# rfahrn/RadVLM

Hardware: AMD Instinct MI355X
Metric: train image-instruction pairs/sec, LLaVA-1.5-7B 336px (higher is better)
Workload: dtype bf16; 1 GPU; llava15_7b full fine-tune step (ViT frozen): fwd+bwd+AdamW, S=704, 32 pairs/GPU/step; global_batch=32, seq_len=704, parallelism=dp1, rows_with_a_label_only=last layer's o_proj / norm / MLP, final norm, lm_head, cross entropy

## Files before the change

include/radvlm_hip.h:

```cpp
#ifndef RADVLM_HIP_H
#define RADVLM_HIP_H
#include <stdint.h>

#ifdef __cplusplus
extern "C" {
#endif

#define RV_ACT_NONE 0
#define RV_ACT_QUICK_GELU 1
#define RV_ACT_GELU 2
#define RV_ACT_GELU_TANH 3

const char* rv_version(void);

int rv_gemm_nt_bf16(const void* A, int64_t lda, const void* B, int64_t ldb, void* C, int64_t ldc, const void* bias,
                    const void* residual, int64_t ldr, int M, int N, int K, int act, int out_f32, int res_f32,
                    const void* zeros16, void* stream);
int rv_gemm_bf16(const void* A, int64_t lda, const void* B, int64_t ldb, void* C, int64_t ldc, const void* bias,
                 const void* residual, int64_t ldr, int M, int N, int K, int trans_a, int trans_b, float alpha, int act,
                 int out_f32, int res_f32, const void* zeros16, void* stream);
int rv_gemm_bf16_ex(const void* A, int64_t lda, const void* B, int64_t ldb, void* C, int64_t ldc, const void* bias,
                    const void* residual, int64_t ldr, int M, int N, int K, int trans_a, int trans_b, float alpha, int act,
                    int out_f32, int res_f32, const void* A2, int64_t lda2, const void* B2, int64_t ldb2, int K2,
                    void* workspace, int64_t workspace_bytes, const void* zeros16, void* stream);
// ... 54 lines not shown
                    int S_pad, int hd, int causal, float scale, void* workspace, int64_t workspace_bytes, const void* zeros16,
                    void* stream);
int rv_attn_bwd_gqa_rope(const void* q, int64_t ld_q, const void* k, int64_t ld_k, const void* v, int64_t ld_v, const void* o,
                         int64_t ld_o, const void* dout, int64_t ld_do, const void* qT, const void* kT, const void* doT,
                         const float* lse, float* delta, void* dq, int64_t ld_dq, void* dk, int64_t ld_dk, void* dv,
                         int64_t ld_dv, const int32_t* lens, const int32_t* cu_rows, int total_rows, int B, int H, int H_kv, int S,
                         int S_pad, int hd, int causal, float scale, void* workspace, int64_t workspace_bytes,
                         const float* rope_cos_sin, const int32_t* rope_positions, const void* zeros16, void* stream);

int rv_attn_bwd_nat(const void* q, int64_t ld_q, const void* k, int64_t ld_k, const void* v, int64_t ld_v, const void* o, int64_t ld_o,
                    const void* dout, int64_t ld_do, const float* lse, float* delta, void* dq, int64_t ld_dq, void* dk, int64_t ld_dk,
                    void* dv, int64_t ld_dv, const int32_t* lens, const int32_t* cu_rows, int total_rows, int B, int H, int H_kv, int S,
                    int S_pad, int hd, int causal, float scale, void* workspace, int64_t workspace_bytes, const float* rope_cos_sin,
                    const int32_t* rope_positions, const void* zeros16, void* stream);

int rv_transpose_bf16_varlen(const void* in, int64_t in_ld, const int32_t* cu_rows, int64_t in_bs1, void* out, int64_t out_ld,
                             int64_t out_bs0, int64_t out_bs1, int R_max, int C, int R_pad, int nb0, int nb1, int perm32,
                             void* stream);
int rv_rope_inplace_pos(void* x, int64_t ld, const float* cos_sin, const int32_t* positions, int rows, int heads, int hd,
                        int nsec, int dir, void* stream);

int rv_swiglu_fwd(const void* gu, int64_t ld_gu, void* act, int64_t ld_act, int rows, int F, void* stream);
int rv_swiglu_bwd(const void* dact, int64_t ld_dact, const void* gu, int64_t ld_gu, void* dgu, int64_t ld_dgu, int rows,
                  int F, void* stream);
int rv_dropout_bf16(const void* x, void* y, int64_t n, float p, uint64_t seed, void* stream);
int rv_dropout_add_bf16(const void* x, void* y, int64_t n, float p, uint64_t seed, void* stream);
int rv_gemm_dropout_add_bf16(const void* A, int64_t lda, const void* B, int64_t ldb, void* C, int64_t ldc, int M, int N, int K, int trans_b,
                             float alpha, float p, uint64_t seed, int accumulate, const void* zeros16, void* stream);
int rv_lora_down_bf16(const void* X, int64_t ldx, const void* A, int64_t lda, void* T, int64_t ldt, int M, int R, int K, float alpha,
                      float p, uint64_t seed, const void* zeros16, void* stream);
// ... 66 lines not shown
```

radvlm_amd/csrc/attention.hip:

```cpp
#include <type_traits>
#include <stdlib.h>
#include "common.h"
#include "radvlm_hip.h"

struct AttnParams {
    const bf16 *q, *k, *v, *o, *dout;
    const bf16 *qT, *kT, *vT, *doT;
    bf16 *out, *dq, *dk, *dv;
    float *lse, *delta;
    const int* lens;
    const int* cu;
    const bf16* zeros;
    long ld_q, ld_k, ld_v, ld_o, ld_do, ld_dq, ld_dk, ld_dv;
    int B, H, S, S_pad;
    int kdiv, qrep;
    int Hkv, nrep;
    float scale;
    const float* rope_cs; const int* rope_pos;
    int paired;
    int rope_dk;
};

namespace {

// ... 54 lines not shown
    return __builtin_amdgcn_make_buffer_rsrc((void*)base, 0, (unsigned)(rows * row_stride * 2), 0x00020000);
}

DEVINL bf16x8 tf_get(const TFrag& f) {
    typedef __attribute__((ext_vector_type(8))) short s16x8n;
    const s16x8n r = {f.t0[0], f.t0[1], f.t0[2], f.t0[3], f.t1[0], f.t1[1], f.t1[2], f.t1[3]};
    return __builtin_bit_cast(bf16x8, r);
}
template <int LEFT> DEVINL void lds_wait8(bf16x8 (&a)[4], bf16x8 (&b)[4]) {
    asm volatile("s_waitcnt lgkmcnt(%8)" : "+v"(a[0]), "+v"(a[1]), "+v"(a[2]), "+v"(a[3]), "+v"(b[0]), "+v"(b[1]), "+v"(b[2]), "+v"(b[3]) : "i"(LEFT) : "memory");
}
template <int LEFT> DEVINL void tf_wait8(TFrag (&f)[4], TFrag (&h)[4]) {
    asm volatile("s_waitcnt lgkmcnt(%16)" : "+v"(f[0].t0), "+v"(f[0].t1), "+v"(f[1].t0), "+v"(f[1].t1), "+v"(f[2].t0), "+v"(f[2].t1), "+v"(f[3].t0), "+v"(f[3].t1),
                   "+v"(h[0].t0), "+v"(h[0].t1), "+v"(h[1].t0), "+v"(h[1].t1), "+v"(h[2].t0), "+v"(h[2].t1), "+v"(h[3].t0), "+v"(h[3].t1) : "i"(LEFT) : "memory");
}
template <int LEFT> DEVINL void tf_wait4(TFrag (&f)[4]) {
    asm volatile("s_waitcnt lgkmcnt(%8)" : "+v"(f[0].t0), "+v"(f[0].t1), "+v"(f[1].t0), "+v"(f[1].t1), "+v"(f[2].t0), "+v"(f[2].t1), "+v"(f[3].t0), "+v"(f[3].t1)
                 : "i"(LEFT) : "memory");
}

template <bool HEAVY_LAST_FIRST>
DEVINL void block_coords(int& xb, int& h, int& b) {
    const int gx = gridDim.x, gy = gridDim.y;
    const int lin = blockIdx.x + gx * (blockIdx.y + gy * blockIdx.z);
    const int pid = xcd_remap(lin, gx * gy * (int)gridDim.z);
    const int hh = pid / gx;
    xb = pid - hh * gx;
    if (HEAVY_LAST_FIRST) xb = gx - 1 - xb;
    h = hh % gy;
    b = hh / gy;
}

template <int N, class F>
DEVINL void sfor(F&& f) {
    if constexpr (N > 0) {
        sfor<N - 1>(f);
        f(std::integral_constant<int, N - 1>{});
    }
}
struct NatAddr {
    unsigned row[4], col[8];
    DEVINL void init(const char* image, int lane) {
        const int g = lane >> 4, c = lane & 15, r1 = (lane >> 2) & 15, pp = lane & 3;
        const unsigned b = lds_off(image);
#pragma unroll
        for (int ks = 0; ks < 4; ++ks) row[ks] = b + c * 256 + (((ks * 4 + g) ^ nswz(c)) << 4);
#pragma unroll
        for (int db = 0; db < 8; ++db) col[db] = b + r1 * 256 + (((2 * db + (pp >> 1)) ^ nswz(r1)) << 4) + ((pp & 1) << 3);
    }
    DEVINL void shift(int delta) {
#pragma unroll
        for (int i = 0; i < 4; ++i) row[i] += delta;
#pragma unroll
        for (int i = 0; i < 8; ++i) col[i] += delta;
    }
};
template <int IMM> DEVINL void rdrow_imm(bf16x8& dst, unsigned a) {
    asm volatile("ds_read_b128 %0, %1 offset:%2" : "=v"(dst) : "v"(a), "i"(IMM) : "memory");
}
template <int IMM> DEVINL void rdcol_imm(TFrag& f, unsigned a) {
    asm volatile("ds_read_b64_tr_b16 %0, %1 offset:%2" : "=v"(f.t0) : "v"(a), "i"(IMM) : "memory");
    asm volatile("ds_read_b64_tr_b16 %0, %1 offset:%2" : "=v"(f.t1) : "v"(a), "i"(IMM + 4096) : "memory");
}
DEVINL float max3_asm(float a, float b, float c) { float r; asm volatile("v_max3_f32 %0, %1, %2, %3" : "=v"(r) : "v"(a), "v"(b), "v"(c)); return r; }

template <int ROW_BYTES> DEVINL int swz(int r) { return ROW_BYTES == 128 ? ((r >> 1) & 7) : (r & 15); }

template <int ROW_BYTES, int NROWS, int NW = 4>
DEVINL void stage_rows(const bf16* src, long row_stride, int valid_rows, const bf16* zeros, char* lds, int wid, int lane) {
    constexpr int CPR = ROW_BYTES / 16;
// ... 619 lines not shown
    for (; t < ntiles; ++t) tile(t, std::false_type{});
#pragma unroll
    for (int qs = 0; qs < 2; ++qs) {
        const int qidx = q0 + qs * 16 + c;
        if (qidx >= S) continue;
        bf16* op = P.dq + (rb + qidx) * P.ld_dq + h * HD + 4 * g;
        f32x4 v[DB];
#pragma unroll
        for (int db = 0; db < DB; ++db) v[db] = dq[qs][db] * P.scale;
        if (P.rope_cs) unrope<DB>(v, P.rope_cs + (long)(P.rope_pos ? P.rope_pos[rb + qidx] : qidx) * HD, g);
#pragma unroll
        for (int db = 0; db < DB; ++db) *(bf16x4*)(op + db * 16) = bf16x4{f2bf(v[db][0]), f2bf(v[db][1]), f2bf(v[db][2]), f2bf(v[db][3])};
    }
}

template <bool CAUSAL, int NW>
__global__ __launch_bounds__(NW * 64, 2) void attn_bwd_dkv_nat_kernel(AttnParams P) {
    constexpr int HD = 128, KS = 4, DB = 8, TILE = 64 * 256, STAGE = 2 * TILE + 1024;
    extern __shared__ __attribute__((aligned(16))) char smem[];
    const int wid = wave_id(), lane = lane_id(), g = lane >> 4, c = lane & 15;
    int kblk, h, b;
    block_coords<false>(kblk, h, b);
    constexpr int KPB = NW * 16;
    const long rb = P.cu ? (long)P.cu[b] : (long)b * P.S;
    const int S = P.cu ? P.cu[b + 1] - P.cu[b] : P.S, k0 = kblk * KPB + wid * 16;
    if (kblk * KPB >= S) return;
    const int len = (P.lens && !P.cu) ? P.lens[b] : S;
    const float sl2 = P.scale * LOG2E;

    bf16x8 kf[KS], vf[KS];
    {
        const int row = min(k0 + c, S - 1);
        const bf16* kp = P.k + (rb + row) * P.ld_k + (h / P.kdiv) * HD + g * 8;
        const bf16* vp = P.v + (rb + row) * P.ld_v + (h / P.kdiv) * HD + g * 8;
#pragma unroll
        for (int ks = 0; ks < KS; ++ks) { kf[ks] = *(const bf16x8*)(kp + ks * 32); vf[ks] = *(const bf16x8*)(vp + ks * 32); }
    }
    const int q_end = len;
    const int t0 = CAUSAL ? (kblk * KPB) >> 6 : 0;
    const int t1 = (q_end + 63) >> 6;
    const int nt = max(t1 - t0, 0);
    const int n_it = nt * P.qrep;

    f32x4 dv[DB], dk[DB];
#pragma unroll
    for (int db = 0; db < DB; ++db) { dv[db] = f32x4{0.f, 0.f, 0.f, 0.f}; dk[db] = f32x4{0.f, 0.f, 0.f, 0.f}; }

    const __amdgpu_buffer_rsrc_t rsQ = rows_rsrc(P.q + rb * P.ld_q, S, P.ld_q), rsO = rows_rsrc(P.dout + rb * P.ld_do, S, P.ld_do);
    NatPlan<64, NW> plQ, plO;
    plQ.init(P.ld_q, wid, lane);
    plO.init(P.ld_do, wid, lane);
    auto stage = [&](int it, char* dst) {
        const int hq = h * P.qrep + it / nt;
        const int qt0 = (t0 + it % nt) * 64;
        const float* lsebase = P.lse + (long)(b * P.H + hq) * P.S_pad;
        const float* dlbase = P.delta + (long)(b * P.H + hq) * P.S_pad;
        plQ.stage(rsQ, (int)((long)qt0 * P.ld_q * 2) + hq * HD * 2, dst, wid);
        plO.stage(rsO, (int)((long)qt0 * P.ld_do * 2) + hq * HD * 2, dst + TILE, wid);
        if (wid == 0) {
            const float* gp = lane < 16 ? lsebase + qt0 + lane * 4 : (lane < 32 ? dlbase + qt0 + (lane - 16) * 4 : (const float*)P.zeros);
            glds16(gp, dst + 2 * TILE);
        }
    };
    if (n_it > 0) stage(0, smem);
    NatAddr ad;
    ad.init(smem + STAGE, lane);

    auto iter = [&](int it, int j, auto edge_tag) {
        constexpr bool EDGE = decltype(edge_tag)::value;
        asm volatile("s_waitcnt vmcnt(0)" ::: "memory");
        __syncthreads();
        ad.shift((it & 1) ? STAGE : -STAGE);
        const char* LSt = smem + (it & 1) * STAGE + 2 * TILE;
        if (it + 1 < n_it) stage(it + 1, smem + ((it + 1) & 1) * STAGE);
        const int qt0 = (t0 + j) * 64;
        if (EDGE && CAUSAL && qt0 + 63 < k0) return;
        {
            sfor<2>([&](auto qpt) {
                constexpr int qp = decltype(qpt)::value;
                if (EDGE && CAUSAL && qt0 + qp * 32 + 31 < k0) return;
                TFrag dc[2][4], qc[2][4];
                auto issue_c = [&](auto bit, TFrag (&dd)[4], TFrag (&qd)[4]) {
                    constexpr int bi = decltype(bit)::value;
                    sfor<4>([&](auto u) {
                        rdcol_imm<TILE + qp * 8192>(dd[decltype(u)::value], ad.col[bi * 4 + decltype(u)::value]);
                        rdcol_imm<qp * 8192>(qd[decltype(u)::value], ad.col[bi * 4 + decltype(u)::value]);
                    });
                };
                f32x4 s[2], dp[2];
                s[0] = s[1] = dp[0] = dp[1] = f32x4{0.f, 0.f, 0.f, 0.f};
                bf16x8 qa[2][KS], da[2][KS];
                sfor<2>([&](auto qq) {
                    sfor<KS>([&](auto ks) {
                        rdrow_imm<(2 * qp + decltype(qq)::value) * 4096>(qa[decltype(qq)::value][decltype(ks)::value], ad.row[decltype(ks)::value]);
                        rdrow_imm<TILE + (2 * qp + decltype(qq)::value) * 4096>(da[decltype(qq)::value][decltype(ks)::value], ad.row[decltype(ks)::value]);
                    });
                });
                lds_wait8<2 * KS>(qa[0], da[0]);
                __builtin_amdgcn_sched_barrier(0);
#pragma unroll
                for (int ks = 0; ks < KS; ++ks) { s[0] = mfma16(qa[0][ks], kf[ks], s[0]); dp[0] = mfma16(da[0][ks], vf[ks], dp[0]); }
                __builtin_amdgcn_sched_barrier(0);
                issue_c(std::integral_constant<int, 0>{}, dc[0], qc[0]);
                lds_wait8<15>(qa[1], da[1]);
                __builtin_amdgcn_sched_barrier(0);
#pragma unroll
                for (int ks = 0; ks < KS; ++ks) { s[1] = mfma16(qa[1][ks], kf[ks], s[1]); dp[1] = mfma16(da[1][ks], vf[ks], dp[1]); }
                __builtin_amdgcn_sched_barrier(0);
#pragma unroll
                for (int qq = 0; qq < 2; ++qq) {
                    const int qrow = qt0 + (2 * qp + qq) * 16 + 4 * g;
                    const f32x4 ls = *(const f32x4*)(LSt + (qrow - qt0) * 4);
                    const f32x4 dl = *(const f32x4*)(LSt + 256 + (qrow - qt0) * 4);
                    const int kidx = k0 + c;
#pragma unroll
                    for (int r = 0; r < 4; ++r) {
                        float p = fexp2(__builtin_fmaf(s[qq][r], sl2, -ls[r] * LOG2E));
                        if (EDGE) {
                            const int qidx = qrow + r;
                            p = ((kidx < len) && (qidx < q_end) && (!CAUSAL || kidx <= qidx)) ? p : 0.f;
                        }
                        s[qq][r] = p;
                        dp[qq][r] = p * (dp[qq][r] - dl[r]);
                    }
                }
                const bf16x8 pf = pack8(s[0], s[1]), dsf = pack8(dp[0], dp[1]);
                sfor<2>([&](auto bit) {
                    constexpr int bi = decltype(bit)::value;
                    if constexpr (bi == 0) { issue_c(std::integral_constant<int, 1>{}, dc[1], qc[1]); tf_wait8<15>(dc[0], qc[0]); }
                    else tf_wait8<0>(dc[1], qc[1]);
                    __builtin_amdgcn_sched_barrier(0);
#pragma unroll
                    for (int u = 0; u < 4; ++u) {
                        dv[bi * 4 + u] = mfma16(tf_get(dc[bi][u]), pf, dv[bi * 4 + u]);
                        dk[bi * 4 + u] = mfma16(tf_get(qc[bi][u]), dsf, dk[bi * 4 + u]);
                    }
                    __builtin_amdgcn_sched_barrier(0);
                });
            });
        }
    };
    {
        const bool key_partial = kblk * KPB + KPB > len;
        const int ne0 = key_partial ? nt : (CAUSAL ? min(nt, (KPB + 63) / 64) : 0);
        const int ni = max(ne0, min(nt, (q_end >> 6) - t0));
        int it = 0;
        for (int rep = 0; rep < P.qrep; ++rep) {
            for (int j = 0; j < ne0; ++j, ++it) iter(it, j, std::true_type{});
            for (int j = ne0; j < ni; ++j, ++it) iter(it, j, std::false_type{});
            for (int j = ni; j < nt; ++j, ++it) iter(it, j, std::true_type{});
        }
    }
    {
        const int kidx = k0 + c;
        if (kidx < S) {
            bf16* vp = P.dv + (rb + kidx) * P.ld_dv + h * HD + 4 * g;
            bf16* kp = P.dk + (rb + kidx) * P.ld_dk + h * HD + 4 * g;
            f32x4 kk[DB];
#pragma unroll
            for (int db = 0; db < DB; ++db) kk[db] = dk[db] * P.scale;
            if (P.rope_cs && P.rope_dk) unrope<DB>(kk, P.rope_cs + (long)(P.rope_pos ? P.rope_pos[rb + kidx] : kidx) * HD, g);
#pragma unroll
            for (int db = 0; db < DB; ++db) {
                const f32x4 a = dv[db];
                *(bf16x4*)(vp + db * 16) = bf16x4{f2bf(a[0]), f2bf(a[1]), f2bf(a[2]), f2bf(a[3])};
                *(bf16x4*)(kp + db * 16) = bf16x4{f2bf(kk[db][0]), f2bf(kk[db][1]), f2bf(kk[db][2]), f2bf(kk[db][3])};
            }
        }
    }
}

template <int HD, bool CAUSAL, int NW>
__global__ __launch_bounds__(NW * 64, NW / 4) void attn_bwd_dq_kernel(AttnParams P) {
    constexpr int KS = HD / 32, DB = HD / 16, KROW = HD * 2;
    constexpr int NAT_BYTES = 64 * KROW, T_BYTES = HD * 128, STAGE = 2 * NAT_BYTES + T_BYTES;
    extern __shared__ __attribute__((aligned(16))) char smem[];
    const int wid = wave_id(), lane = lane_id(), g = lane >> 4, c = lane & 15;
    const int qblk = blockIdx.x, h = blockIdx.y, b = blockIdx.z;
    const long rb = P.cu ? (long)P.cu[b] : (long)b * P.S;
// ... 315 lines not shown
    } while (0)
    if (HD == 128) { if (causal) LAUNCH_FWD(128, true); else LAUNCH_FWD(128, false); }
    else { if (causal) LAUNCH_FWD(64, true); else LAUNCH_FWD(64, false); }
#undef LAUNCH_FWD
    return rv_check_launch();
}

namespace {
template __global__ void attn_fwd_nat_kernel<true>(AttnParams);
template __global__ void attn_fwd_nat_kernel<false>(AttnParams);
#ifndef RV_DQ_NW
#define RV_DQ_NW 4
#endif
template __global__ void attn_bwd_dq_nat_kernel<true, RV_DQ_NW>(AttnParams);
template __global__ void attn_bwd_dq_nat_kernel<false, RV_DQ_NW>(AttnParams);
template __global__ void attn_bwd_dkv_nat_kernel<true, 4>(AttnParams);
template __global__ void attn_bwd_dkv_nat_kernel<false, 4>(AttnParams);
}

static int g_attn_cus() {
    static int cus = 0;
    if (!cus) {
        int dev = 0, n = 0;
        if (hipGetDevice(&dev) == hipSuccess && hipDeviceGetAttribute(&n, hipDeviceAttributeMultiprocessorCount, dev) == hipSuccess && n > 0) cus = n;
        else cus = 256;
    }
    return cus;
}
static int attn_fwd_pairs(int B, int H, int S, int causal) {
    const int nq = (S + 127) / 128;
    const long pairs = (long)((nq + 1) / 2) * H * B;
    const long slots = 2L * g_attn_cus();
// ... 80 lines not shown
    } while (0)
    if (HD == 128) { if (causal) LAUNCH_BWD(128, true); else LAUNCH_BWD(128, false); }
    else { if (causal) LAUNCH_BWD(64, true); else LAUNCH_BWD(64, false); }
#undef LAUNCH_BWD
    if (expand) {
        const long rows = rows_all, total = rows * (H_kv * HD / 16);
        hipLaunchKernelGGL(group_sum_heads_kernel, dim3((total + 255) / 256), dim3(256), 0, st, PK.dk, PK.ld_dk, P.dk, P.ld_dk, rows, H_kv, P.nrep, HD,
                           rope_cos_sin, rope_positions, cu_rows, S);
        hipLaunchKernelGGL(group_sum_heads_kernel, dim3((total + 255) / 256), dim3(256), 0, st, PK.dv, PK.ld_dv, P.dv, P.ld_dv, rows, H_kv, P.nrep, HD,
                           (const float*)nullptr, (const int32_t*)nullptr, cu_rows, S);
    }
    return rv_check_launch();
}


extern "C" int rv_attn_bwd_nat(const void* q, int64_t ld_q, const void* k, int64_t ld_k, const void* v, int64_t ld_v, const void* o, int64_t ld_o,
                               const void* dout, int64_t ld_do, const float* lse, float* delta, void* dq, int64_t ld_dq, void* dk, int64_t ld_dk,
                               void* dv, int64_t ld_dv, const int32_t* lens, const int32_t* cu_rows, int total_rows, int B, int H, int H_kv, int S,
                               int S_pad, int HD, int causal, float scale, void* workspace, int64_t workspace_bytes, const float* rope_cos_sin,
                               const int32_t* rope_positions, const void* zeros16, void* stream) {
    if (!q || !k || !v || !o || !dout || !lse || !delta || !dq || !dk || !dv || !zeros16) return RV_ERR_ARG;
    if (H_kv <= 0 || H <= 0 || H % H_kv || HD != 128 || (S_pad & 63) || S_pad < S || B <= 0 || S <= 0) return RV_ERR_ARG;
    if ((ld_q & 7) || (ld_k & 7) || (ld_v & 7) || (ld_do & 7) || (ld_o & 7) || (ld_dq & 3) || (ld_dk & 3) || (ld_dv & 3)) return RV_ERR_ARG;
    if (!aligned_ok(q) || !aligned_ok(k) || !aligned_ok(v) || !aligned_ok(dout) || !aligned_ok(o)) return RV_ERR_ARG;
    if (rope_cos_sin && ((((uintptr_t)rope_cos_sin) & 15) || (cu_rows && !rope_positions))) return RV_ERR_ARG;
    AttnParams P = {};
    P.q = (const bf16*)q; P.k = (const bf16*)k; P.v = (const bf16*)v; P.o = (const bf16*)o; P.dout = (const bf16*)dout;
    P.dq = (bf16*)dq; P.dk = (bf16*)dk; P.dv = (bf16*)dv; P.lse = (float*)lse; P.delta = delta; P.lens = lens; P.cu = cu_rows;
    P.zeros = (const bf16*)zeros16;
    P.ld_q = ld_q; P.ld_k = ld_k; P.ld_v = ld_v; P.ld_o = ld_o; P.ld_do = ld_do; P.ld_dq = ld_dq; P.ld_dk = ld_dk; P.ld_dv = ld_dv;
    P.B = B; P.H = H; P.S = S; P.S_pad = S_pad; P.scale = scale; P.Hkv = H_kv; P.nrep = H / H_kv;
    P.rope_cs = rope_cos_sin; P.rope_pos = rope_positions; P.rope_dk = 1;
    hipStream_t st = (hipStream_t)stream;
    dim3 grid_dq((S + 32 * RV_DQ_NW - 1) / (32 * RV_DQ_NW), H, B), grid_dkv((S + 63) / 64, H_kv, B);
    AttnParams PK = P;
    PK.kdiv = 1; PK.qrep = P.nrep;
    const long rows_all = cu_rows ? (long)total_rows : (long)B * S;
    if (cu_rows && total_rows <= 0) return RV_ERR_ARG;
    const int64_t need = 2 * (int64_t)rows_all * H * HD * 2;
    const bool expand = P.nrep > 1 && workspace && workspace_bytes >= need && (((uintptr_t)workspace) & 15) == 0 &&
                        (long)grid_dkv.x * H_kv * B < 4096;
    if (expand) {
        PK.kdiv = P.nrep; PK.qrep = 1; PK.rope_dk = 0;
        PK.dk = (bf16*)workspace; PK.dv = (bf16*)workspace + (int64_t)rows_all * H * HD;
        PK.ld_dk = PK.ld_dv = (long)H * HD;
        grid_dkv.y = H;
    }
    const int smem_dq = 2 * 2 * 64 * 256, smem_dkv = 2 * (2 * 64 * 256 + 1024);
#define LAUNCH_BWD_NAT(C_)                                                                                 \
    do {                                                                                                   \
        set_smem(attn_bwd_dq_nat_kernel<C_, RV_DQ_NW>, smem_dq);                                                  \
        set_smem(attn_bwd_dkv_nat_kernel<C_, 4>, smem_dkv);                                                \
        hipLaunchKernelGGL((attn_bwd_dq_nat_kernel<C_, RV_DQ_NW>), grid_dq, dim3(64 * RV_DQ_NW), smem_dq, st, P);           \
        hipLaunchKernelGGL((attn_bwd_dkv_nat_kernel<C_, 4>), grid_dkv, dim3(256), smem_dkv, st, PK);       \
    } while (0)
    if (causal) LAUNCH_BWD_NAT(true); else LAUNCH_BWD_NAT(false);
#undef LAUNCH_BWD_NAT
    if (expand) {
        const long total = rows_all * (H_kv * HD / 16);
        hipLaunchKernelGGL(group_sum_heads_kernel, dim3((total + 255) / 256), dim3(256), 0, st, PK.dk, PK.ld_dk, P.dk, P.ld_dk, rows_all, H_kv, P.nrep, HD,
                           rope_cos_sin, rope_positions, cu_rows, S);
        hipLaunchKernelGGL(group_sum_heads_kernel, dim3((total + 255) / 256), dim3(256), 0, st, PK.dv, PK.ld_dv, P.dv, P.ld_dv, rows_all, H_kv, P.nrep, HD,
                           (const float*)nullptr, (const int32_t*)nullptr, cu_rows, S);
    }
    return rv_check_launch();
}

extern "C" int rv_attn_bwd_gqa(const void* q, int64_t ld_q, const void* k, int64_t ld_k, const void* v, int64_t ld_v,
                               const void* o, int64_t ld_o, const void* dout, int64_t ld_do, const void* qT, const void* kT,
                               const void* doT, const float* lse, float* delta, void* dq, int64_t ld_dq, void* dk,
                               int64_t ld_dk, void* dv, int64_t ld_dv, const int32_t* lens, const int32_t* cu_rows, int total_rows,
                               int B, int H, int H_kv, int S, int S_pad, int HD, int causal, float scale, void* workspace, int64_t workspace_bytes,
                               const void* zeros16, void* stream) {
    return rv_attn_bwd_gqa_rope(q, ld_q, k, ld_k, v, ld_v, o, ld_o, dout, ld_do, qT, kT, doT, lse, delta, dq, ld_dq, dk, ld_dk, dv, ld_dv,
                                lens, cu_rows, total_rows, B, H, H_kv, S, S_pad, HD, causal, scale, workspace, workspace_bytes, nullptr, nullptr,
                                zeros16, stream);
}

extern "C" int rv_attn_bwd(const void* q, int64_t ld_q, const void* k, int64_t ld_k, const void* v, int64_t ld_v,
                           const void* o, int64_t ld_o, const void* dout, int64_t ld_do, const void* qT, const void* kT,
// ... 7 lines not shown
```

radvlm_amd/lib.py:

```python
import ctypes
import os

import torch

_HERE = os.path.dirname(os.path.abspath(__file__))
_LIB_PATH = os.path.join(_HERE, "libradvlm_hip.so")

_c_void_p = ctypes.c_void_p
_i64 = ctypes.c_int64
_i32 = ctypes.c_int
_f32 = ctypes.c_float

ACT_NONE, ACT_QUICK_GELU, ACT_GELU, ACT_GELU_TANH = 0, 1, 2, 3

_SIGS = {
    "rv_gemm_nt_bf16": [_c_void_p, _i64, _c_void_p, _i64, _c_void_p, _i64, _c_void_p, _c_void_p, _i64, _i32, _i32, _i32,
                        _i32, _i32, _i32, _c_void_p, _c_void_p],
    "rv_gemm_bf16": [_c_void_p, _i64, _c_void_p, _i64, _c_void_p, _i64, _c_void_p, _c_void_p, _i64, _i32, _i32, _i32, _i32, _i32,
                     _f32, _i32, _i32, _i32, _c_void_p, _c_void_p],
    "rv_gemm_bf16_ex": [_c_void_p, _i64, _c_void_p, _i64, _c_void_p, _i64, _c_void_p, _c_void_p, _i64, _i32, _i32, _i32, _i32, _i32,
                        _f32, _i32, _i32, _i32, _c_void_p, _i64, _c_void_p, _i64, _i32, _c_void_p, _i64, _c_void_p, _c_void_p],
    "rv_gemm_rope_bf16": [_c_void_p, _i64, _c_void_p, _i64, _c_void_p, _i64, _c_void_p, _i32, _i32, _i32, _c_void_p, _c_void_p, _i32, _i32, _i32,
                          _c_void_p, _i64, _c_void_p, _c_void_p],
    "rv_gemm_swiglu_fwd_bf16": [_c_void_p, _i64, _c_void_p, _i64, _c_void_p, _i64, _c_void_p, _i64, _i32, _i32, _i32, _c_void_p, _i64, _c_void_p,
# ... 19 lines not shown
    "rv_attn_fwd": [_c_void_p, _i64, _c_void_p, _i64, _c_void_p, _c_void_p, _i64, _c_void_p, _c_void_p, _i32, _i32, _i32, _i32,
                    _i32, _i32, _f32, _c_void_p, _c_void_p],
    "rv_attn_bwd": [_c_void_p, _i64, _c_void_p, _i64, _c_void_p, _i64, _c_void_p, _i64, _c_void_p, _i64, _c_void_p, _c_void_p,
                    _c_void_p, _c_void_p, _c_void_p, _c_void_p, _i64, _c_void_p, _i64, _c_void_p, _i64, _c_void_p, _i32, _i32,
                    _i32, _i32, _i32, _i32, _f32, _c_void_p, _c_void_p],
    "rv_attn_fwd_gqa": [_c_void_p, _i64, _c_void_p, _i64, _c_void_p, _c_void_p, _i64, _c_void_p, _c_void_p, _c_void_p, _i32, _i32, _i32,
                        _i32, _i32, _i32, _i32, _f32, _c_void_p, _c_void_p],
    "rv_attn_bwd_gqa": [_c_void_p, _i64, _c_void_p, _i64, _c_void_p, _i64, _c_void_p, _i64, _c_void_p, _i64, _c_void_p, _c_void_p,
                        _c_void_p, _c_void_p, _c_void_p, _c_void_p, _i64, _c_void_p, _i64, _c_void_p, _i64, _c_void_p, _c_void_p, _i32,
                        _i32, _i32, _i32, _i32, _i32, _i32, _i32, _f32, _c_void_p, _i64, _c_void_p, _c_void_p],
    "rv_attn_fwd_nat": [_c_void_p, _i64, _c_void_p, _i64, _c_void_p, _i64, _c_void_p, _i64, _c_void_p, _c_void_p, _c_void_p, _i32, _i32, _i32,
                        _i32, _i32, _i32, _i32, _f32, _c_void_p, _c_void_p],
    "rv_attn_bwd_nat": [_c_void_p, _i64, _c_void_p, _i64, _c_void_p, _i64, _c_void_p, _i64, _c_void_p, _i64, _c_void_p, _c_void_p, _c_void_p, _i64,
                        _c_void_p, _i64, _c_void_p, _i64, _c_void_p, _c_void_p, _i32, _i32, _i32, _i32, _i32, _i32, _i32, _i32, _f32, _c_void_p, _i64,
                        _c_void_p, _c_void_p, _c_void_p, _c_void_p],
    "rv_attn_bwd_gqa_rope": [_c_void_p, _i64, _c_void_p, _i64, _c_void_p, _i64, _c_void_p, _i64, _c_void_p, _i64, _c_void_p, _c_void_p,
                             _c_void_p, _c_void_p, _c_void_p, _c_void_p, _i64, _c_void_p, _i64, _c_void_p, _i64, _c_void_p, _c_void_p, _i32,
                             _i32, _i32, _i32, _i32, _i32, _i32, _i32, _f32, _c_void_p, _i64, _c_void_p, _c_void_p, _c_void_p, _c_void_p],
    "rv_transpose_bf16_varlen": [_c_void_p, _i64, _c_void_p, _i64, _c_void_p, _i64, _i64, _i64, _i32, _i32, _i32, _i32, _i32, _i32,
                                 _c_void_p],
    "rv_rope_inplace_pos": [_c_void_p, _i64, _c_void_p, _c_void_p, _i32, _i32, _i32, _i32, _i32, _c_void_p],
    "rv_gelu_tanh_fwd": [_c_void_p, _c_void_p, _i64, _c_void_p],
    "rv_gelu_tanh_bwd": [_c_void_p, _c_void_p, _c_void_p, _i64, _c_void_p],
    "rv_weighted_segment_sum_rows": [_c_void_p, _i64, _c_void_p, _c_void_p, _c_void_p, _c_void_p, _i32, _c_void_p, _i64, _i32,
                                     _c_void_p],
    "rv_max4_rows_fwd": [_c_void_p, _i64, _c_void_p, _c_void_p, _i32, _c_void_p, _i64, _c_void_p, _i32, _c_void_p],
    "rv_max4_rows_bwd": [_c_void_p, _i64, _c_void_p, _c_void_p, _i32, _c_void_p, _c_void_p, _i64, _i32, _c_void_p],
    "rv_add_pos_rows": [_c_void_p, _c_void_p, _i32, _i32, _i32, _c_void_p],
    "rv_swiglu_fwd": [_c_void_p, _i64, _c_void_p, _i64, _i32, _i32, _c_void_p],
    "rv_swiglu_bwd": [_c_void_p, _i64, _c_void_p, _i64, _c_void_p, _i64, _i32, _i32, _c_void_p],
# ... 88 lines not shown
```

radvlm_amd/ops.py:

```python
import math

import torch

from . import lib
from .lib import ACT_GELU, ACT_GELU_TANH, ACT_NONE, ACT_QUICK_GELU

BF16 = torch.bfloat16


def _chk(t, dtype=BF16):
    assert t.is_cuda and t.dtype == dtype, (t.device, t.dtype)
    return t


def round_up(x, m):
    return (x + m - 1) // m * m


_WS = {}


def default_workspace(device):
    key = (device.type, device.index)
    if key not in _WS:
# ... 248 lines not shown
    if out is None:
        out = torch.empty(q.shape[0], H * hd, dtype=BF16, device=q.device)
    if lse is None:
        lse = torch.zeros(B, H, s_pad, dtype=torch.float32, device=q.device)
    if v is not None:
        assert vT is None and hd == 128
        lib.call("rv_attn_fwd_nat", q, q.stride(0), k, k.stride(0), v, v.stride(0), out, out.stride(0), lse, lens, cu, B, H, Hkv, S, s_pad, hd,
                 int(causal), scale, lib.zeros16(q.device))
        return out, lse
    lib.call("rv_attn_fwd_gqa", q, q.stride(0), k, k.stride(0), vT, out, out.stride(0), lse, lens, cu, B, H, Hkv, S, s_pad, hd,
             int(causal), scale, lib.zeros16(q.device))
    return out, lse


def attn_bwd(q, k, v, o, dout, lse, B, S, H, hd, s_pad, causal, lens=None, scale=None, dq=None, dk=None, dv=None,
             kv_heads=None, use_workspace=True, cu=None, rope=None, natural=True, delta=None):
    scale = scale if scale is not None else 1.0 / math.sqrt(hd)
    dev = q.device
    Hkv = kv_heads or H
    rows = q.shape[0]
    if hd == 128 and natural:
        delta = torch.zeros(B, H, s_pad, dtype=torch.float32, device=dev) if delta is None else delta
        dq = torch.empty(rows, H * hd, dtype=BF16, device=dev) if dq is None else dq
        dk = torch.empty(rows, Hkv * hd, dtype=BF16, device=dev) if dk is None else dk
        dv = torch.empty(rows, Hkv * hd, dtype=BF16, device=dev) if dv is None else dv
        ws = torch.empty(2 * rows * H * hd, dtype=BF16, device=dev) if (Hkv != H and use_workspace) else None
        lib.call("rv_attn_bwd_nat", q, q.stride(0), k, k.stride(0), v, v.stride(0), o, o.stride(0), dout, dout.stride(0), lse, delta,
                 dq, dq.stride(0), dk, dk.stride(0), dv, dv.stride(0), lens, cu, rows if cu is not None else 0, B, H, Hkv, S, s_pad, hd,
                 int(causal), scale, ws, ws.numel() * ws.element_size() if ws is not None else 0,
                 rope[0] if rope else None, rope[1] if rope else None, lib.zeros16(dev))
        return dq, dk, dv
    qT = transpose_heads(q, B, S, H, hd, s_pad, cu=cu)
    kT = transpose_heads(k, B, S, Hkv, hd, s_pad, cu=cu)
    doT = transpose_heads(dout, B, S, H, hd, s_pad, cu=cu)
    delta = torch.zeros(B, H, s_pad, dtype=torch.float32, device=dev) if delta is None else delta
    dq = torch.empty(rows, H * hd, dtype=BF16, device=dev) if dq is None else dq
    dk = torch.empty(rows, Hkv * hd, dtype=BF16, device=dev) if dk is None else dk
    dv = torch.empty(rows, Hkv * hd, dtype=BF16, device=dev) if dv is None else dv
    ws = torch.empty(2 * rows * H * hd, dtype=BF16, device=dev) if (Hkv != H and use_workspace) else None
    lib.call("rv_attn_bwd_gqa_rope", q, q.stride(0), k, k.stride(0), v, v.stride(0), o, o.stride(0), dout, dout.stride(0), qT, kT, doT,
             lse, delta, dq, dq.stride(0), dk, dk.stride(0), dv, dv.stride(0), lens, cu, rows if cu is not None else 0, B, H, Hkv, S,
             s_pad, hd, int(causal), scale,
             ws, ws.numel() * ws.element_size() if ws is not None else 0, rope[0] if rope else None, rope[1] if rope else None, lib.zeros16(dev))
    return dq, dk, dv

# ... 329 lines not shown
```

Baseline: 42.85 pairs/s.

## Let dK/dV attention backward waves own 32 keys to reuse Q/dO LDS reads

Templates the natural-layout dK/dV backward kernel on keys-per-wave, adding a 32-key variant. In that variant each wave keeps two 16-key groups of K/V fragments and accumulators, and each Q/dO fragment read from LDS feeds MFMAs for both groups, using a new XOR-swizzled address helper. A heuristic picks 32 keys per wave when there are enough 128-key blocks to fill the CUs, which halves the dK/dV grid. The aim is to cut LDS traffic and per-block staging overhead per key. The cost is more accumulator and fragment registers, which may hurt occupancy, and coarser causal skipping.

```diff
diff --git a/include/radvlm_hip.h b/include/radvlm_hip.h
--- a/include/radvlm_hip.h
+++ b/include/radvlm_hip.h
@@ -92,6 +92,12 @@
                     int S_pad, int hd, int causal, float scale, void* workspace, int64_t workspace_bytes, const float* rope_cos_sin,
                     const int32_t* rope_positions, const void* zeros16, void* stream);
 
+int rv_attn_bwd_nat_kpw(const void* q, int64_t ld_q, const void* k, int64_t ld_k, const void* v, int64_t ld_v, const void* o, int64_t ld_o,
+                        const void* dout, int64_t ld_do, const float* lse, float* delta, void* dq, int64_t ld_dq, void* dk, int64_t ld_dk,
+                        void* dv, int64_t ld_dv, const int32_t* lens, const int32_t* cu_rows, int total_rows, int B, int H, int H_kv, int S,
+                        int S_pad, int hd, int causal, float scale, void* workspace, int64_t workspace_bytes, const float* rope_cos_sin,
+                        const int32_t* rope_positions, int keys_per_wave, const void* zeros16, void* stream);
+
 int rv_transpose_bf16_varlen(const void* in, int64_t in_ld, const int32_t* cu_rows, int64_t in_bs1, void* out, int64_t out_ld,
                              int64_t out_bs0, int64_t out_bs1, int R_max, int C, int R_pad, int nb0, int nb1, int perm32,
                              void* stream);
diff --git a/radvlm_amd/csrc/attention.hip b/radvlm_amd/csrc/attention.hip
--- a/radvlm_amd/csrc/attention.hip
+++ b/radvlm_amd/csrc/attention.hip
@@ -92,6 +92,9 @@
     asm volatile("s_waitcnt lgkmcnt(%16)" : "+v"(f[0].t0), "+v"(f[0].t1), "+v"(f[1].t0), "+v"(f[1].t1), "+v"(f[2].t0), "+v"(f[2].t1), "+v"(f[3].t0), "+v"(f[3].t1),
                    "+v"(h[0].t0), "+v"(h[0].t1), "+v"(h[1].t0), "+v"(h[1].t1), "+v"(h[2].t0), "+v"(h[2].t1), "+v"(h[3].t0), "+v"(h[3].t1) : "i"(LEFT) : "memory");
 }
+template <int LEFT> DEVINL void tf_wait2(TFrag& f, TFrag& h) {
+    asm volatile("s_waitcnt lgkmcnt(%4)" : "+v"(f.t0), "+v"(f.t1), "+v"(h.t0), "+v"(h.t1) : "i"(LEFT) : "memory");
+}
 template <int LEFT> DEVINL void tf_wait4(TFrag (&f)[4]) {
     asm volatile("s_waitcnt lgkmcnt(%8)" : "+v"(f[0].t0), "+v"(f[0].t1), "+v"(f[1].t0), "+v"(f[1].t1), "+v"(f[2].t0), "+v"(f[2].t1), "+v"(f[3].t0), "+v"(f[3].t1)
                  : "i"(LEFT) : "memory");
@@ -109,6 +112,11 @@
     b = hh / gy;
 }
 
+DEVINL int lane_id_again() {
+    int l;
+    asm volatile("v_mbcnt_lo_u32_b32 %0, -1, 0\n\tv_mbcnt_hi_u32_b32 %0, -1, %0" : "=v"(l));
+    return l;
+}
 template <int N, class F>
 DEVINL void sfor(F&& f) {
     if constexpr (N > 0) {
@@ -132,6 +140,18 @@
 #pragma unroll
         for (int i = 0; i < 8; ++i) col[i] += delta;
     }
+};
+struct NatAddrXor {
+    unsigned r, c;
+    DEVINL void init(const char* image, int lane) {
+        const int g = lane >> 4, cc = lane & 15, r1 = (lane >> 2) & 15, pp = lane & 3;
+        const unsigned b = lds_off(image);
+        r = b + cc * 256 + ((g ^ nswz(cc)) << 4);
+        c = b + r1 * 256 + (((pp >> 1) ^ nswz(r1)) << 4) + ((pp & 1) << 3);
+    }
+    DEVINL void shift(int delta) { r += delta; c += delta; }
+    template <int KS> DEVINL unsigned row() const { return r ^ (KS << 6); }
+    template <int DB> DEVINL unsigned col() const { return c ^ (DB << 5); }
 };
 template <int IMM> DEVINL void rdrow_imm(bf16x8& dst, unsigned a) {
     asm volatile("ds_read_b128 %0, %1 offset:%2" : "=v"(dst) : "v"(a), "i"(IMM) : "memory");
@@ -781,27 +801,31 @@
     }
 }
 
-template <bool CAUSAL, int NW>
+template <bool CAUSAL, int NW, int KPW>
 __global__ __launch_bounds__(NW * 64, 2) void attn_bwd_dkv_nat_kernel(AttnParams P) {
+    static_assert(KPW == 16 || KPW == 32, "16 or 32 keys per wave");
     constexpr int HD = 128, KS = 4, DB = 8, TILE = 64 * 256, STAGE = 2 * TILE + 1024;
-    extern __shared__ __attribute__((aligned(16))) char smem[];
+    constexpr int NG = KPW / 16;
+    extern __shared__ __attribute__((aligned(1024))) char smem_dkv[];
+    char* const smem = smem_dkv;
     const int wid = wave_id(), lane = lane_id(), g = lane >> 4, c = lane & 15;
     int kblk, h, b;
     block_coords<false>(kblk, h, b);
-    constexpr int KPB = NW * 16;
+    constexpr int KPB = NW * KPW;
     const long rb = P.cu ? (long)P.cu[b] : (long)b * P.S;
-    const int S = P.cu ? P.cu[b + 1] - P.cu[b] : P.S, k0 = kblk * KPB + wid * 16;
+    const int S = P.cu ? P.cu[b + 1] - P.cu[b] : P.S, k0 = kblk * KPB + wid * KPW;
     if (kblk * KPB >= S) return;
     const int len = (P.lens && !P.cu) ? P.lens[b] : S;
     const float sl2 = P.scale * LOG2E;
 
-    bf16x8 kf[KS], vf[KS];
-    {
-        const int row = min(k0 + c, S - 1);
+    bf16x8 kf[NG][KS], vf[NG][KS];
+#pragma unroll
+    for (int kg = 0; kg < NG; ++kg) {
+        const int row = min(k0 + kg * 16 + c, S - 1);
         const bf16* kp = P.k + (rb + row) * P.ld_k + (h / P.kdiv) * HD + g * 8;
         const bf16* vp = P.v + (rb + row) * P.ld_v + (h / P.kdiv) * HD + g * 8;
 #pragma unroll
-        for (int ks = 0; ks < KS; ++ks) { kf[ks] = *(const bf16x8*)(kp + ks * 32); vf[ks] = *(const bf16x8*)(vp + ks * 32); }
+        for (int ks = 0; ks < KS; ++ks) { kf[kg][ks] = *(const bf16x8*)(kp + ks * 32); vf[kg][ks] = *(const bf16x8*)(vp + ks * 32); }
     }
     const int q_end = len;
     const int t0 = CAUSAL ? (kblk * KPB) >> 6 : 0;
@@ -809,15 +833,17 @@
     const int nt = max(t1 - t0, 0);
     const int n_it = nt * P.qrep;
 
-    f32x4 dv[DB], dk[DB];
-#pragma unroll
-    for (int db = 0; db < DB; ++db) { dv[db] = f32x4{0.f, 0.f, 0.f, 0.f}; dk[db] = f32x4{0.f, 0.f, 0.f, 0.f}; }
+    f32x4 dv[NG][DB], dk[NG][DB];
+#pragma unroll
+    for (int kg = 0; kg < NG; ++kg)
+#pragma unroll
+        for (int db = 0; db < DB; ++db) { dv[kg][db] = f32x4{0.f, 0.f, 0.f, 0.f}; dk[kg][db] = f32x4{0.f, 0.f, 0.f, 0.f}; }
 
     const __amdgpu_buffer_rsrc_t rsQ = rows_rsrc(P.q + rb * P.ld_q, S, P.ld_q), rsO = rows_rsrc(P.dout + rb * P.ld_do, S, P.ld_do);
-    NatPlan<64, NW> plQ, plO;
-    plQ.init(P.ld_q, wid, lane);
-    plO.init(P.ld_do, wid, lane);
-    auto stage = [&](int it, char* dst) {
+    auto stage = [&](int it, char* dst, int lane) {
+        NatPlan<64, NW> plQ, plO;
+        plQ.init(P.ld_q, wid, lane);
+        plO.init(P.ld_do, wid, lane);
         const int hq = h * P.qrep + it / nt;
         const int qt0 = (t0 + it % nt) * 64;
         const float* lsebase = P.lse + (long)(b * P.H + hq) * P.S_pad;
@@ -829,8 +855,8 @@
             glds16(gp, dst + 2 * TILE);
         }
     };
-    if (n_it > 0) stage(0, smem);
-    NatAddr ad;
+    if (n_it > 0) stage(0, smem, lane);
+    std::conditional_t<NG == 1, NatAddr, NatAddrXor> ad;
     ad.init(smem + STAGE, lane);
 
     auto iter = [&](int it, int j, auto edge_tag) {
@@ -839,13 +865,23 @@
         __syncthreads();
         ad.shift((it & 1) ? STAGE : -STAGE);
         const char* LSt = smem + (it & 1) * STAGE + 2 * TILE;
-        if (it + 1 < n_it) stage(it + 1, smem + ((it + 1) & 1) * STAGE);
+        const int lane = NG == 1 ? lane_id() : lane_id_again(), g = lane >> 4, c = lane & 15;
+        if (it + 1 < n_it) stage(it + 1, smem + ((it + 1) & 1) * STAGE, lane);
         const int qt0 = (t0 + j) * 64;
         if (EDGE && CAUSAL && qt0 + 63 < k0) return;
-        {
-            sfor<2>([&](auto qpt) {
-                constexpr int qp = decltype(qpt)::value;
-                if (EDGE && CAUSAL && qt0 + qp * 32 + 31 < k0) return;
+        auto p_ds = [&](f32x4& s, f32x4& dp, const f32x4 ls, const f32x4 dl, int q0, int kb) {
+#pragma unroll
+            for (int r = 0; r < 4; ++r) {
+                float p = fexp2(__builtin_fmaf(s[r], sl2, -ls[r] * LOG2E));
+                if (EDGE) p = ((c < len - kb) & (4 * g < q_end - q0 - r) & (!CAUSAL || c - 4 * g <= q0 + r - kb)) ? p : 0.f;
+                s[r] = p;
+                dp[r] = p * (dp[r] - dl[r]);
+            }
+        };
+        sfor<2>([&](auto qpt) {
+            constexpr int qp = decltype(qpt)::value;
+            if (NG == 1 && EDGE && CAUSAL && qt0 + qp * 32 + 31 < k0) return;
+            if constexpr (NG == 1) {
                 TFrag dc[2][4], qc[2][4];
                 auto issue_c = [&](auto bit, TFrag (&dd)[4], TFrag (&qd)[4]) {
                     constexpr int bi = decltype(bit)::value;
@@ -866,30 +902,19 @@
                 lds_wait8<2 * KS>(qa[0], da[0]);
                 __builtin_amdgcn_sched_barrier(0);
 #pragma unroll
-                for (int ks = 0; ks < KS; ++ks) { s[0] = mfma16(qa[0][ks], kf[ks], s[0]); dp[0] = mfma16(da[0][ks], vf[ks], dp[0]); }
+                for (int ks = 0; ks < KS; ++ks) { s[0] = mfma16(qa[0][ks], kf[0][ks], s[0]); dp[0] = mfma16(da[0][ks], vf[0][ks], dp[0]); }
                 __builtin_amdgcn_sched_barrier(0);
                 issue_c(std::integral_constant<int, 0>{}, dc[0], qc[0]);
                 lds_wait8<15>(qa[1], da[1]);
                 __builtin_amdgcn_sched_barrier(0);
 #pragma unroll
-                for (int ks = 0; ks < KS; ++ks) { s[1] = mfma16(qa[1][ks], kf[ks], s[1]); dp[1] = mfma16(da[1][ks], vf[ks], dp[1]); }
+                for (int ks = 0; ks < KS; ++ks) { s[1] = mfma16(qa[1][ks], kf[0][ks], s[1]); dp[1] = mfma16(da[1][ks], vf[0][ks], dp[1]); }
                 __builtin_amdgcn_sched_barrier(0);
 #pragma unroll
                 for (int qq = 0; qq < 2; ++qq) {
-                    const int qrow = qt0 + (2 * qp + qq) * 16 + 4 * g;
-                    const f32x4 ls = *(const f32x4*)(LSt + (qrow - qt0) * 4);
-                    const f32x4 dl = *(const f32x4*)(LSt + 256 + (qrow - qt0) * 4);
-                    const int kidx = k0 + c;
-#pragma unroll
-                    for (int r = 0; r < 4; ++r) {
-                        float p = fexp2(__builtin_fmaf(s[qq][r], sl2, -ls[r] * LOG2E));
-                        if (EDGE) {
-                            const int qidx = qrow + r;
-                            p = ((kidx < len) && (qidx < q_end) && (!CAUSAL || kidx <= qidx)) ? p : 0.f;
-                        }
-                        s[qq][r] = p;
-                        dp[qq][r] = p * (dp[qq][r] - dl[r]);
-                    }
+                    const f32x4 ls = *(const f32x4*)(LSt + ((2 * qp + qq) * 16 + 4 * g) * 4);
+                    const f32x4 dl = *(const f32x4*)(LSt + 256 + ((2 * qp + qq) * 16 + 4 * g) * 4);
+                    p_ds(s[qq], dp[qq], ls, dl, qt0 + (2 * qp + qq) * 16, k0);
                 }
                 const bf16x8 pf = pack8(s[0], s[1]), dsf = pack8(dp[0], dp[1]);
                 sfor<2>([&](auto bit) {
@@ -899,13 +924,71 @@
                     __builtin_amdgcn_sched_barrier(0);
 #pragma unroll
                     for (int u = 0; u < 4; ++u) {
-                        dv[bi * 4 + u] = mfma16(tf_get(dc[bi][u]), pf, dv[bi * 4 + u]);
-                        dk[bi * 4 + u] = mfma16(tf_get(qc[bi][u]), dsf, dk[bi * 4 + u]);
+                        dv[0][bi * 4 + u] = mfma16(tf_get(dc[bi][u]), pf, dv[0][bi * 4 + u]);
+                        dk[0][bi * 4 + u] = mfma16(tf_get(qc[bi][u]), dsf, dk[0][bi * 4 + u]);
                     }
                     __builtin_amdgcn_sched_barrier(0);
                 });
-            });
-        }
+            } else {
+                bf16x8 rq[1], ro[1];
+                TFrag co[2], cq[2];
+                auto issue_r = [&](auto ut) {
+                    constexpr int u = decltype(ut)::value, qq = u / KS, ks = u % KS;
+                    const unsigned a = ad.template row<ks>();
+                    rdrow_imm<(2 * qp + qq) * 4096>(rq[0], a);
+                    rdrow_imm<TILE + (2 * qp + qq) * 4096>(ro[0], a);
+                };
+                auto issue_c = [&](auto dbt) {
+                    constexpr int db = decltype(dbt)::value;
+                    const unsigned a = ad.template col<db>();
+                    rdcol_imm<TILE + qp * 8192>(co[db & 1], a);
+                    rdcol_imm<qp * 8192>(cq[db & 1], a);
+                };
+                bf16x4 ph[NG][2], dh[NG][2];
+                sfor<2>([&](auto qqt) {
+                    constexpr int qq = decltype(qqt)::value;
+                    f32x4 s[NG], dp[NG];
+#pragma unroll
+                    for (int kg = 0; kg < NG; ++kg) s[kg] = dp[kg] = f32x4{0.f, 0.f, 0.f, 0.f};
+                    sfor<KS>([&](auto kst) {
+                        constexpr int ks = decltype(kst)::value, u = qq * KS + ks;
+                        issue_r(std::integral_constant<int, u>{});
+                        lds_wait2<0>(rq[0], ro[0]);
+                        __builtin_amdgcn_sched_barrier(0);
+#pragma unroll
+                        for (int kg = 0; kg < NG; ++kg) { s[kg] = mfma16(rq[0], kf[kg][ks], s[kg]); dp[kg] = mfma16(ro[0], vf[kg][ks], dp[kg]); }
+                        __builtin_amdgcn_sched_barrier(0);
+                    });
+                    const f32x4 ls = *(const f32x4*)(LSt + ((2 * qp + qq) * 16 + 4 * g) * 4);
+                    const f32x4 dl = *(const f32x4*)(LSt + 256 + ((2 * qp + qq) * 16 + 4 * g) * 4);
+#pragma unroll
+                    for (int kg = 0; kg < NG; ++kg) {
+                        p_ds(s[kg], dp[kg], ls, dl, qt0 + (2 * qp + qq) * 16, k0 + kg * 16);
+                        ph[kg][qq] = bf16x4{f2bf(s[kg][0]), f2bf(s[kg][1]), f2bf(s[kg][2]), f2bf(s[kg][3])};
+                        dh[kg][qq] = bf16x4{f2bf(dp[kg][0]), f2bf(dp[kg][1]), f2bf(dp[kg][2]), f2bf(dp[kg][3])};
+                        asm volatile("" : "+v"(ph[kg][qq]), "+v"(dh[kg][qq]));
+                        __builtin_amdgcn_sched_barrier(0);
+                    }
+                });
+                issue_c(std::integral_constant<int, 0>{});
+                bf16x8 pf[NG], dsf[NG];
+#pragma unroll
+                for (int kg = 0; kg < NG; ++kg) {
+                    pf[kg] = __builtin_shufflevector(ph[kg][0], ph[kg][1], 0, 1, 2, 3, 4, 5, 6, 7);
+                    dsf[kg] = __builtin_shufflevector(dh[kg][0], dh[kg][1], 0, 1, 2, 3, 4, 5, 6, 7);
+                }
+                sfor<DB>([&](auto dbt) {
+                    constexpr int db = decltype(dbt)::value;
+                    if constexpr (db + 1 < DB) { issue_c(std::integral_constant<int, db + 1>{}); tf_wait2<4>(co[db & 1], cq[db & 1]); }
+                    else tf_wait2<0>(co[db & 1], cq[db & 1]);
+                    __builtin_amdgcn_sched_barrier(0);
+                    const bf16x8 of = tf_get(co[db & 1]), qf = tf_get(cq[db & 1]);
+#pragma unroll
+                    for (int kg = 0; kg < NG; ++kg) { dv[kg][db] = mfma16(of, pf[kg], dv[kg][db]); dk[kg][db] = mfma16(qf, dsf[kg], dk[kg][db]); }
+                    __builtin_amdgcn_sched_barrier(0);
+                });
+            }
+        });
     };
     {
         const bool key_partial = kblk * KPB + KPB > len;
@@ -918,18 +1001,19 @@
             for (int j = ni; j < nt; ++j, ++it) iter(it, j, std::true_type{});
         }
     }
-    {
-        const int kidx = k0 + c;
+#pragma unroll
+    for (int kg = 0; kg < NG; ++kg) {
+        const int kidx = k0 + kg * 16 + c;
         if (kidx < S) {
             bf16* vp = P.dv + (rb + kidx) * P.ld_dv + h * HD + 4 * g;
             bf16* kp = P.dk + (rb + kidx) * P.ld_dk + h * HD + 4 * g;
             f32x4 kk[DB];
 #pragma unroll
-            for (int db = 0; db < DB; ++db) kk[db] = dk[db] * P.scale;
+            for (int db = 0; db < DB; ++db) kk[db] = dk[kg][db] * P.scale;
             if (P.rope_cs && P.rope_dk) unrope<DB>(kk, P.rope_cs + (long)(P.rope_pos ? P.rope_pos[rb + kidx] : kidx) * HD, g);
 #pragma unroll
             for (int db = 0; db < DB; ++db) {
-                const f32x4 a = dv[db];
+                const f32x4 a = dv[kg][db];
                 *(bf16x4*)(vp + db * 16) = bf16x4{f2bf(a[0]), f2bf(a[1]), f2bf(a[2]), f2bf(a[3])};
                 *(bf16x4*)(kp + db * 16) = bf16x4{f2bf(kk[db][0]), f2bf(kk[db][1]), f2bf(kk[db][2]), f2bf(kk[db][3])};
             }
@@ -1275,8 +1359,10 @@
 #endif
 template __global__ void attn_bwd_dq_nat_kernel<true, RV_DQ_NW>(AttnParams);
 template __global__ void attn_bwd_dq_nat_kernel<false, RV_DQ_NW>(AttnParams);
-template __global__ void attn_bwd_dkv_nat_kernel<true, 4>(AttnParams);
-template __global__ void attn_bwd_dkv_nat_kernel<false, 4>(AttnParams);
+template __global__ void attn_bwd_dkv_nat_kernel<true, 4, 16>(AttnParams);
+template __global__ void attn_bwd_dkv_nat_kernel<false, 4, 16>(AttnParams);
+template __global__ void attn_bwd_dkv_nat_kernel<true, 4, 32>(AttnParams);
+template __global__ void attn_bwd_dkv_nat_kernel<false, 4, 32>(AttnParams);
 }
 
 static int g_attn_cus() {
@@ -1387,11 +1473,17 @@
 }
 
 
-extern "C" int rv_attn_bwd_nat(const void* q, int64_t ld_q, const void* k, int64_t ld_k, const void* v, int64_t ld_v, const void* o, int64_t ld_o,
+#ifndef RV_DKV_KPW
+#define RV_DKV_KPW 0
+#endif
+static int attn_dkv_kpw(long n128) { return RV_DKV_KPW ? RV_DKV_KPW : (n128 >= 2L * g_attn_cus() ? 32 : 16); }
+
+extern "C" int rv_attn_bwd_nat_kpw(const void* q, int64_t ld_q, const void* k, int64_t ld_k, const void* v, int64_t ld_v, const void* o, int64_t ld_o,
                                const void* dout, int64_t ld_do, const float* lse, float* delta, void* dq, int64_t ld_dq, void* dk, int64_t ld_dk,
                                void* dv, int64_t ld_dv, const int32_t* lens, const int32_t* cu_rows, int total_rows, int B, int H, int H_kv, int S,
                                int S_pad, int HD, int causal, float scale, void* workspace, int64_t workspace_bytes, const float* rope_cos_sin,
-                               const int32_t* rope_positions, const void* zeros16, void* stream) {
+                               const int32_t* rope_positions, int keys_per_wave, const void* zeros16, void* stream) {
+    if (keys_per_wave != 0 && keys_per_wave != 16 && keys_per_wave != 32) return RV_ERR_ARG;
     if (!q || !k || !v || !o || !dout || !lse || !delta || !dq || !dk || !dv || !zeros16) return RV_ERR_ARG;
     if (H_kv <= 0 || H <= 0 || H % H_kv || HD != 128 || (S_pad & 63) || S_pad < S || B <= 0 || S <= 0) return RV_ERR_ARG;
     if ((ld_q & 7) || (ld_k & 7) || (ld_v & 7) || (ld_do & 7) || (ld_o & 7) || (ld_dq & 3) || (ld_dk & 3) || (ld_dv & 3)) return RV_ERR_ARG;
@@ -1420,15 +1512,23 @@
         grid_dkv.y = H;
     }
     const int smem_dq = 2 * 2 * 64 * 256, smem_dkv = 2 * (2 * 64 * 256 + 1024);
+    const int n128 = (S + 127) / 128;
+    const int kpw = keys_per_wave ? keys_per_wave : attn_dkv_kpw((long)n128 * grid_dkv.y * B);
+    if (kpw == 32) grid_dkv.x = n128;
+#define LAUNCH_DKV_NAT(C_, KPW_)                                                                           \
+    do {                                                                                                   \
+        set_smem(attn_bwd_dkv_nat_kernel<C_, 4, KPW_>, smem_dkv);                                          \
+        hipLaunchKernelGGL((attn_bwd_dkv_nat_kernel<C_, 4, KPW_>), grid_dkv, dim3(256), smem_dkv, st, PK); \
+    } while (0)
 #define LAUNCH_BWD_NAT(C_)                                                                                 \
     do {                                                                                                   \
         set_smem(attn_bwd_dq_nat_kernel<C_, RV_DQ_NW>, smem_dq);                                                  \
-        set_smem(attn_bwd_dkv_nat_kernel<C_, 4>, smem_dkv);                                                \
         hipLaunchKernelGGL((attn_bwd_dq_nat_kernel<C_, RV_DQ_NW>), grid_dq, dim3(64 * RV_DQ_NW), smem_dq, st, P);           \
-        hipLaunchKernelGGL((attn_bwd_dkv_nat_kernel<C_, 4>), grid_dkv, dim3(256), smem_dkv, st, PK);       \
+        if (kpw == 32) LAUNCH_DKV_NAT(C_, 32); else LAUNCH_DKV_NAT(C_, 16);                                \
     } while (0)
     if (causal) LAUNCH_BWD_NAT(true); else LAUNCH_BWD_NAT(false);
 #undef LAUNCH_BWD_NAT
+#undef LAUNCH_DKV_NAT
     if (expand) {
         const long total = rows_all * (H_kv * HD / 16);
         hipLaunchKernelGGL(group_sum_heads_kernel, dim3((total + 255) / 256), dim3(256), 0, st, PK.dk, PK.ld_dk, P.dk, P.ld_dk, rows_all, H_kv, P.nrep, HD,
@@ -1437,6 +1537,15 @@
                            (const float*)nullptr, (const int32_t*)nullptr, cu_rows, S);
     }
     return rv_check_launch();
+}
+
+extern "C" int rv_attn_bwd_nat(const void* q, int64_t ld_q, const void* k, int64_t ld_k, const void* v, int64_t ld_v, const void* o, int64_t ld_o,
+                               const void* dout, int64_t ld_do, const float* lse, float* delta, void* dq, int64_t ld_dq, void* dk, int64_t ld_dk,
+                               void* dv, int64_t ld_dv, const int32_t* lens, const int32_t* cu_rows, int total_rows, int B, int H, int H_kv, int S,
+                               int S_pad, int HD, int causal, float scale, void* workspace, int64_t workspace_bytes, const float* rope_cos_sin,
+                               const int32_t* rope_positions, const void* zeros16, void* stream) {
+    return rv_attn_bwd_nat_kpw(q, ld_q, k, ld_k, v, ld_v, o, ld_o, dout, ld_do, lse, delta, dq, ld_dq, dk, ld_dk, dv, ld_dv, lens, cu_rows, total_rows,
+                               B, H, H_kv, S, S_pad, HD, causal, scale, workspace, workspace_bytes, rope_cos_sin, rope_positions, 0, zeros16, stream);
 }
 
 extern "C" int rv_attn_bwd_gqa(const void* q, int64_t ld_q, const void* k, int64_t ld_k, const void* v, int64_t ld_v,
diff --git a/radvlm_amd/lib.py b/radvlm_amd/lib.py
--- a/radvlm_amd/lib.py
+++ b/radvlm_amd/lib.py
@@ -57,6 +57,9 @@
     "rv_attn_bwd_nat": [_c_void_p, _i64, _c_void_p, _i64, _c_void_p, _i64, _c_void_p, _i64, _c_void_p, _i64, _c_void_p, _c_void_p, _c_void_p, _i64,
                         _c_void_p, _i64, _c_void_p, _i64, _c_void_p, _c_void_p, _i32, _i32, _i32, _i32, _i32, _i32, _i32, _i32, _f32, _c_void_p, _i64,
                         _c_void_p, _c_void_p, _c_void_p, _c_void_p],
+    "rv_attn_bwd_nat_kpw": [_c_void_p, _i64, _c_void_p, _i64, _c_void_p, _i64, _c_void_p, _i64, _c_void_p, _i64, _c_void_p, _c_void_p, _c_void_p, _i64,
+                            _c_void_p, _i64, _c_void_p, _i64, _c_void_p, _c_void_p, _i32, _i32, _i32, _i32, _i32, _i32, _i32, _i32, _f32, _c_void_p, _i64,
+                            _c_void_p, _c_void_p, _i32, _c_void_p, _c_void_p],
     "rv_attn_bwd_gqa_rope": [_c_void_p, _i64, _c_void_p, _i64, _c_void_p, _i64, _c_void_p, _i64, _c_void_p, _i64, _c_void_p, _c_void_p,
                              _c_void_p, _c_void_p, _c_void_p, _c_void_p, _i64, _c_void_p, _i64, _c_void_p, _i64, _c_void_p, _c_void_p, _i32,
                              _i32, _i32, _i32, _i32, _i32, _i32, _i32, _f32, _c_void_p, _i64, _c_void_p, _c_void_p, _c_void_p, _c_void_p],
diff --git a/radvlm_amd/ops.py b/radvlm_amd/ops.py
--- a/radvlm_amd/ops.py
+++ b/radvlm_amd/ops.py
@@ -286,7 +286,7 @@
 
 
 def attn_bwd(q, k, v, o, dout, lse, B, S, H, hd, s_pad, causal, lens=None, scale=None, dq=None, dk=None, dv=None,
-             kv_heads=None, use_workspace=True, cu=None, rope=None, natural=True, delta=None):
+             kv_heads=None, use_workspace=True, cu=None, rope=None, natural=True, delta=None, keys_per_wave=0):
     scale = scale if scale is not None else 1.0 / math.sqrt(hd)
     dev = q.device
     Hkv = kv_heads or H
@@ -297,10 +297,14 @@
         dk = torch.empty(rows, Hkv * hd, dtype=BF16, device=dev) if dk is None else dk
         dv = torch.empty(rows, Hkv * hd, dtype=BF16, device=dev) if dv is None else dv
         ws = torch.empty(2 * rows * H * hd, dtype=BF16, device=dev) if (Hkv != H and use_workspace) else None
-        lib.call("rv_attn_bwd_nat", q, q.stride(0), k, k.stride(0), v, v.stride(0), o, o.stride(0), dout, dout.stride(0), lse, delta,
-                 dq, dq.stride(0), dk, dk.stride(0), dv, dv.stride(0), lens, cu, rows if cu is not None else 0, B, H, Hkv, S, s_pad, hd,
-                 int(causal), scale, ws, ws.numel() * ws.element_size() if ws is not None else 0,
-                 rope[0] if rope else None, rope[1] if rope else None, lib.zeros16(dev))
+        args = (q, q.stride(0), k, k.stride(0), v, v.stride(0), o, o.stride(0), dout, dout.stride(0), lse, delta,
+                dq, dq.stride(0), dk, dk.stride(0), dv, dv.stride(0), lens, cu, rows if cu is not None else 0, B, H, Hkv, S, s_pad, hd,
+                int(causal), scale, ws, ws.numel() * ws.element_size() if ws is not None else 0,
+                rope[0] if rope else None, rope[1] if rope else None)
+        if keys_per_wave:
+            lib.call("rv_attn_bwd_nat_kpw", *args, int(keys_per_wave), lib.zeros16(dev))
+        else:
+            lib.call("rv_attn_bwd_nat", *args, lib.zeros16(dev))
         return dq, dk, dv
     qT = transpose_heads(q, B, S, H, hd, s_pad, cu=cu)
     kT = transpose_heads(k, B, S, Hkv, hd, s_pad, cu=cu)
```

Result: no change. 42.79 pairs/s, median of 3 (-0.1%).
